# google/zopfli

Measured on AMD Instinct MI355X. Metric: input MB/s at numiterations=15 (gzip, bit-exact vs reference), higher is better.
Workload: dtype u8 (f32/f64 cost DP); 1 GPU; class-T synthetic (text-like, the enwik8 stand-in) 100000000 B per GPU, numiterations=15, blocksplitting=0, gzip, BASELINE configs[1]; total_bytes=100000000, master_blocks=100, gather=none (one rank)

## Files before the change

include/zopfli_amd.h:

```cpp
#ifndef ZOPFLI_AMD_H_
#define ZOPFLI_AMD_H_

#include <stddef.h>
#include <stdint.h>

#ifdef __cplusplus
extern "C" {
#endif

#if defined(__GNUC__)
#pragma GCC visibility push(default)
#endif



typedef struct ZopfliOptions {
  int verbose;
  int verbose_more;
  int numiterations;
  int blocksplitting;
  int blocksplittinglast;
  int blocksplittingmax;
} ZopfliOptions;

// ... 164 lines not shown
int zmx_master_block_costs(const unsigned char* in, size_t insize, double* cost, size_t ncost);
int zmx_deal_master_blocks(const double* cost, size_t nblocks, size_t shards, size_t* first);

int zmx_last_timing(double* out8);

int zmx_last_kernel_timing(double* out4);
void zmx_set_kernel_timing(int on);

int zmx_last_host_timing(double* out2);

int zmx_last_match_timing(double* out4);
int zmx_last_match_walk(double* out3);

typedef void (*zmx_oom_hook_t)(int device);
void zmx_set_oom_hook(zmx_oom_hook_t hook);
int zmx_ctx_set_share(zmx_ctx* ctx, unsigned contexts_on_device);
int zmx_ctx_trim_cache(zmx_ctx* ctx);
int zmx_ctx_set_priority(zmx_ctx* ctx, int level);

int zmx_set_match_kernel(int kernel);

int zmx_last_seg_stats(double* out8);

#if defined(__GNUC__)
#pragma GCC visibility pop
#endif

#ifdef __cplusplus
}
#endif

#endif
```

zopfli_amd/api.py:

```python
import ctypes
import os

from ._build import LIB

if os.environ.get("ZOPFLI_AMD_LIB"):
    LIB = os.environ["ZOPFLI_AMD_LIB"]

FORMAT_GZIP, FORMAT_ZLIB, FORMAT_DEFLATE = 0, 1, 2
CRC32, ADLER32 = 0, 1
ZMX_HIST = 320


class ZopfliOptions(ctypes.Structure):
    _fields_ = [("verbose", ctypes.c_int), ("verbose_more", ctypes.c_int), ("numiterations", ctypes.c_int),
                ("blocksplitting", ctypes.c_int), ("blocksplittinglast", ctypes.c_int),
                ("blocksplittingmax", ctypes.c_int)]

    def __init__(self, numiterations=15, blocksplitting=1, blocksplittingmax=15, verbose=0, verbose_more=0):
        super().__init__(verbose, verbose_more, numiterations, blocksplitting, 0, blocksplittingmax)


class ZmxBlock(ctypes.Structure):
    _fields_ = [("instart", ctypes.c_uint64), ("inend", ctypes.c_uint64)]

# ... 160 lines not shown
    k = (ctypes.c_double * 4)()
    lib.zmx_last_kernel_timing(k)
    d["wtab_kernel"], d["trace_kernel"] = k[0], k[2]
    h = (ctypes.c_double * 2)()
    lib.zmx_last_host_timing(h)
    d["download"], d["serialize"] = h[0], h[1]
    m = (ctypes.c_double * 4)()
    lib.zmx_last_match_timing(m)
    d["match_kernel"], d["hash_kernels"], d["table_builds"], d["positions_matched"] = m[0], m[1], m[2], m[3]
    w = (ctypes.c_double * 3)()
    lib.zmx_last_match_walk(w)
    d["skip_walk_lane_iterations"], d["skip_walk_wave_iterations"], d["skip_walk_positions"] = w[0], w[1], w[2]
    return d


def last_seg_stats(lib=None):
    lib = lib or library()
    t = (ctypes.c_double * 8)()
    lib.zmx_last_seg_stats(t)
    keys = ["tasks", "accepted", "rerun_state", "rerun_level", "rerun_tie", "positions_rerun", "rerun_values", "positions"]
    return dict(zip(keys, list(t)))


class Context:

    def __init__(self, device=0, lib=None):
        self.lib = lib or library()
        self.handle = ctypes.c_void_p()
        self._input = None
        self._segments = None
        if self.lib.zmx_ctx_create(device, ctypes.byref(self.handle)) != 0:
            raise RuntimeError("zmx_ctx_create: " + self.error())

    def error(self):
        return (self.lib.zmx_last_error() or b"").decode()

    def _check(self, rc, what):
        if rc != 0:
            raise RuntimeError(f"{what}: {self.error()}")

    def close(self):
        if self.handle:
            self.lib.zmx_ctx_destroy(self.handle)
            self.handle = ctypes.c_void_p()

    def set_input(self, data):
# ... 316 lines not shown
```

zopfli_amd/csrc/device/zmx_dp4.h:

```cpp
#pragma once

#define D3_RELAX_K(CS, LT, WV, K)                                            \
  {                                                                          \
    const double old_ = (double)(CS);                                        \
    const double nc_ = (WV) + cj;                                            \
    LT = nc_ < old_ ? (K) : LT;                                              \
    CS = (float)fmin(nc_, old_);                                             \
  }

#define D3_ROT32()                                                           \
  {                                                                          \
    if (reach < 64) {                    \
      c[0] = __uint_as_float(__builtin_amdgcn_permlane32_swap(__float_as_uint(c[0]), __float_as_uint(1e30f), false, false)[1]); \
      l[0] = __builtin_amdgcn_permlane32_swap(l[0], 0u, false, false)[1];    \
    } else {                                                                 \
      d3_rot32(c, l, lane);                                                  \
    }                                                                        \
    reach = reach >= 32 ? reach - 32 : 0;                                    \
  }

#define D4_TRACK_MAX() { vmax = fmaxf(vmax, c[0] < 1e29f ? c[0] : 0.0f); }

#define D3_RETIRE32(WB)                                                      \
  {                                                                          \
// ... 216 lines not shown
  u64* prof;
  const u32* badpos;
  const SegTask* tasks;
  const u32* task_off;
  float* lvl;
  const float* est_bits;
  SegSnap* entry;
  SegSnap* exit;
  SegSnap* mid;
  SegCheck* chk;
  const float* wmax;
  const u32* tiemask;
  u32* stats;
  float level_scale;
  const u32* wg_tasks;
  const u32* wmeta;
  const u32* winroff;
  const u32* winflag;
  const u32* win_off;
  int debug;
  u16* over;
  u32* redo_count;
  u32* redo_wg;
  int int_path;
  int fix_lean_min;
  int redo_pass;
  int chain_fast;
  int coop;
  const u32* kind;
  const u32* run_list;
  u32* flags;
};

struct D4Job {
  u32 cell = 0;
  u32 start;
  u32 noshort;
  u32 pout;
  u32 pend;
  u32 la_lo;
  u32 over_lo;
  bool spec;
  bool load;
  float level;
  double delta;
  const SegSnap* init;
// ... 486 lines not shown
            }
          }
        }
      }
      const u64 tk1 = D3_TICK();
      __syncthreads();
      if (PROF) { tq[2] += tk1 - tk0; tq[3] += D3_TICK() - tk1; }
      ++it;
      if (last) break;
    }
    __syncthreads();
    if (PROF && P.prof && wave == 2 && lane == 0) {
      u64* o = P.prof + (u64)b * ZMX_PROF_N + 24;
      for (int i = 0; i < 4; ++i) atomicAdd(&o[i], tq[i]);
    }
  }
#undef D3_TICK
  __builtin_amdgcn_fence(__ATOMIC_RELEASE, "agent");
  __syncthreads();
  __builtin_amdgcn_fence(__ATOMIC_ACQUIRE, "agent");
}

__global__ __launch_bounds__(64) void k_dpcheck(Dp4Params P) {
  if (blockIdx.x == 0 && threadIdx.x == 0) *P.redo_count = 0;
  const u32 t = P.task0 + blockIdx.x;
  if (P.tasks[t].pout == 0) return;
  const SegCheck r = d4_check(&P.exit[t - 1], &P.entry[t], threadIdx.x);
  if (threadIdx.x == 0) P.chk[t] = r;
}

__device__ __forceinline__ u32 d4_accept(float vmin, double vmax, double delta, double wmax, u32 tiemask) {
  if (delta == 0.0) return 0;
  const int e = (int)((__float_as_uint(vmin) >> 23) & 255u) - 127;
  const double lo = ldexp(1.0, e), hi = ldexp(1.0, e + 1);
  const bool pure = vmin >= 16.0f && vmax + wmax < hi && (double)vmin + delta >= lo && vmax + wmax + delta < hi;
  if (!pure) return 1;
  return ((tiemask >> (e & 31)) & 1u) != 0 ? 2u : 0u;
}

__global__ __launch_bounds__(64) void k_dpscan(Dp4Params P) {
  const u32 b = P.block0 + blockIdx.x;
  const u32 t0 = P.task_off[b], t1 = P.task_off[b + 1];
  const u32 lane = threadIdx.x;
  const double wmax = (double)P.wmax[b] + 1.0;
  const u32 tiemask = P.tiemask[b];
  double carry = 0.0;
  for (u32 c0 = t0 + 1; c0 < t1; c0 += 64) {
    const u32 t = c0 + lane;
    const bool act = t < t1;
    SegCheck ck;
    ck.d = 0.0; ck.vmin = 0.0f; ck.match = 0;
// ... 31 lines not shown
```

zopfli_amd/csrc/device/zmx_hip.hip:

```cpp
#include <hip/hip_runtime.h>

#include <algorithm>
#include <atomic>
#include <cmath>
#include <cstdio>
#include <cstdlib>
#include <cstring>
#include <mutex>
#include <string>
#include <unordered_map>
#include <vector>

#include "zmx_kernels.h"
#include "zmx_match2.h"
#ifdef ZMX_EXPERIMENTS
#include "zmx_match3.h"
#include "zmx_match4.h"
#else
#define BK_CH 32768u
#endif
#include "zmx_match5.h"
#include "zmx_dp4.h"
#include "zmx_dp5.h"
#include "zmx_encode.h"
#include "zmx_checksum.h"
#include "zmx_trace.h"
#include "zmx_greedy.h"
#include "zmx_png.h"
#include "zmx_png_brute.h"
#include "zmx_blockcost.h"
#include "zopfli_amd.h"
#include "../host/symbol_check.h"
#include "../host/thread_pool.h"

namespace {

thread_local std::string g_err;
struct ThreadStats {
  double kernel_seconds[3];
  double squeeze_launches;
  double match5[3];
  double match[4];
  double seg[8];
};
static_assert(sizeof(ThreadStats) == 19 * sizeof(double), "zmx_internal_stats_take / _add move 19 doubles");
thread_local ThreadStats g_ts = {};
#define g_kernel_seconds g_ts.kernel_seconds
#define g_squeeze_launches g_ts.squeeze_launches
#define g_match5_stats g_ts.match5
#define g_match_stats g_ts.match
#define g_seg_stats g_ts.seg

thread_local bool g_last_oom = false;
thread_local int g_err_class = ZMX_ERR_NONE;

int Fail(const char* what, hipError_t e, const char* file, int line) {
  char buf[512];
  std::snprintf(buf, sizeof(buf), "%s: %s (%s:%d)", what, hipGetErrorString(e), file, line);
  g_err = buf;
  g_last_oom = e == hipErrorOutOfMemory;
  g_err_class = g_last_oom ? ZMX_ERR_OUT_OF_MEMORY : ZMX_ERR_DEVICE;
  if (g_last_oom) (void)hipGetLastError();
  return -1;
}
int FailMsg(const std::string& m) {
  g_err = m;
  g_err_class = ZMX_ERR_REFUSED;
  return -1;
}
int FailFault(const std::string& m) {
  g_err = m;
  g_err_class = ZMX_ERR_DEVICE;
  return -1;
}
// ... 94 lines not shown
  bool buckets = false;
  u32* d_recs = nullptr;
  u32* d_pool = nullptr;
  u32 pool_cap = 0;
  u16* d_la = nullptr;
  u32* d_store[2] = {nullptr, nullptr};
  u32* d_hist = nullptr;
  u32* d_nsym = nullptr;
  double* d_cost = nullptr;
  double* d_mincost = nullptr;
  int* d_slot = nullptr;
  uint2* d_dph = nullptr;
  u64* d_block_edges = nullptr;
  u32* d_badpos = nullptr;
  size_t badpos_words = 0;
  bool badpos_clean = false;
  u64* d_code_base = nullptr;
  u16* d_codes = nullptr;
  double* d_wtab = nullptr;
  u32* d_badcodes = nullptr;
  u32* d_seg_off = nullptr;
  u32* d_extab = nullptr;
  uint2* d_seginfo = nullptr;
  std::vector<u32> seg_off;
  std::vector<u64> block_edges;
  std::vector<u32> tile_off;
  u32* d_counters = nullptr;
  u32* d_flags = nullptr;
  unsigned char* d_runin = nullptr;
  unsigned char* d_runout = nullptr;
  unsigned char* h_runin = nullptr;
  unsigned char* h_runout = nullptr;
  size_t h_runin_cap = 0, h_runout_cap = 0;
  size_t runin_bytes = 0, runout_bytes = 0;
  u64* d_prof = nullptr;
  std::vector<SegTask> tasks;
  std::vector<u32> task_off;
  SegTask* d_tasks = nullptr;
  u32* d_task_off = nullptr;
  u32* d_wg_tasks = nullptr;
  u32 n_wg = 0;
  u32 n_wg_runs = 0;
  u32* d_task_kind = nullptr;
  u32* d_run_list = nullptr;
  u32 n_run_list = 0;
  u32* d_wmeta = nullptr;
// ... 251 lines not shown
  c->pool_free_bytes = 0;
  return 0;
}

int zmx_set_match_kernel(int kernel) {
#ifdef ZMX_EXPERIMENTS
  if (kernel != 0 && kernel != 2 && kernel != 3 && kernel != 4 && kernel != 5) return FailMsg("zmx_set_match_kernel: 0, 2, 3, 4 or 5");
#else
  if (kernel == 3 || kernel == 4) return FailMsg("zmx_set_match_kernel: kernels 3 and 4 are in -DZMX_EXPERIMENTS builds only");
  if (kernel != 0 && kernel != 2 && kernel != 5) return FailMsg("zmx_set_match_kernel: 0, 2 or 5");
#endif
  g_match_kernel.store(kernel, std::memory_order_relaxed);
  return 0;
}

size_t zmx_internal_input_size(zmx_ctx* ctx) { return ctx->insize; }
int zmx_internal_device(zmx_ctx* ctx) { return ctx->device; }
void zmx_internal_set_error(const char* msg) { g_err = msg; g_err_class = ZMX_ERR_DEVICE; }
void zmx_internal_set_error_class(const char* msg, int cls) { g_err = msg; g_err_class = cls; }
const unsigned char* zmx_internal_input_host(zmx_ctx* ctx) { return ctx->h_in; }

void zmx_internal_seg_stats(double* out8, int reset) {
  for (int i = 0; i < 8; ++i) out8[i] = g_seg_stats[i];
  if (reset) for (int i = 0; i < 8; ++i) g_seg_stats[i] = 0;
}

void zmx_internal_match5_stats(double* out3, int reset) {
  for (int i = 0; i < 3; ++i) out3[i] = g_match5_stats[i];
  if (reset) for (int i = 0; i < 3; ++i) g_match5_stats[i] = 0;
}

void zmx_internal_match_stats(double* out4, int reset) {
  for (int i = 0; i < 4; ++i) out4[i] = g_match_stats[i];
  if (reset) for (int i = 0; i < 4; ++i) g_match_stats[i] = 0;
}

void zmx_internal_kernel_stats(double* seconds3, double* squeeze_launches, int reset) {
  for (int i = 0; i < 3; ++i) seconds3[i] = g_kernel_seconds[i];
  *squeeze_launches = g_squeeze_launches;
  if (reset) {
    g_kernel_seconds[0] = g_kernel_seconds[1] = g_kernel_seconds[2] = 0;
    g_squeeze_launches = 0;
  }
}

void zmx_internal_stats_take(double* out19) {
  std::memcpy(out19, &g_ts, sizeof(g_ts));
  g_ts = ThreadStats{};
}
void zmx_internal_stats_add(const double* in19) {
  double* d = reinterpret_cast<double*>(&g_ts);
  for (int i = 0; i < 19; ++i) d[i] += in19[i];
}

static hipError_t PinnedTake(zmx_ctx* c, unsigned char** p, size_t bytes, size_t* cap) {
  size_t best = c->pinned_free.size();
  for (size_t i = 0; i < c->pinned_free.size(); ++i) {
    const size_t k = c->pinned_free[i].second;
    if (k >= bytes && k <= 4 * bytes + 4096 && (best == c->pinned_free.size() || k < c->pinned_free[best].second)) best = i;
  }
  if (best != c->pinned_free.size()) {
    *p = c->pinned_free[best].first;
    *cap = c->pinned_free[best].second;
    c->pinned_free.erase(c->pinned_free.begin() + static_cast<long>(best));
    return hipSuccess;
  }
  *cap = bytes < 4096 ? 4096 : bytes;
  return hipHostMalloc(reinterpret_cast<void**>(p), *cap, hipHostMallocDefault);
}
static void PinnedGive(zmx_ctx* c, unsigned char** p, size_t cap) {
  if (!*p) return;
  if (c && c->pinned_free.size() < 8 && cap <= (64u << 20)) c->pinned_free.emplace_back(*p, cap);
  else (void)hipHostFree(*p);
  *p = nullptr;
}
// ... 105 lines not shown

static void ReleaseTableArrays(zmx_ctx* c, zmx_tables* t, bool keep_stores) {
  auto rel = [&](auto*& p) { PoolFree(c, p); p = nullptr; };
  rel(t->d_blocks);
  rel(t->d_tile_off);
  rel(t->d_same16);
  rel(t->d_links);
  rel(t->d_sorted_alloc);
  rel(t->d_ssame);
  rel(t->d_chunk_base);
  rel(t->d_recs);
  rel(t->d_pool);
  rel(t->d_la);
  rel(t->d_dph);
  rel(t->d_block_edges);
  rel(t->d_badpos);
  rel(t->d_code_base);
  rel(t->d_codes);
  rel(t->d_wtab);
  rel(t->d_badcodes);
  rel(t->d_seg_off);
  rel(t->d_extab);
  rel(t->d_seginfo);
  rel(t->d_counters);
  rel(t->d_prof);
  rel(t->d_tasks);
  rel(t->d_task_off);
  rel(t->d_wg_tasks);
  rel(t->d_task_kind);
  rel(t->d_run_list);
  rel(t->d_wmeta);
  rel(t->d_runin);
  rel(t->d_runout);
  rel(t->d_winroff);
  rel(t->d_winflag);
  rel(t->d_win_off);
  rel(t->d_lvl);
  rel(t->d_entry);
  rel(t->d_exit);
  rel(t->d_mid);
  rel(t->d_chk);
  rel(t->d_over);
  rel(t->d_redo);
  for (int h = 0; h < 2; ++h) { rel(t->d_rank[h]); rel(t->d_bucket[h]); }
  t->d_sorted[0] = t->d_sorted[1] = nullptr;
  PinnedGive(c, &t->h_runin, t->h_runin_cap);
// ... 16 lines not shown
  HIPCHK(hipStreamSynchronize(c->stream));
  HIPCHK(hipStreamSynchronize(c->stream2));
  ReleaseTableArrays(c, t, true);
  t->trimmed = true;
  return 0;
}

static unsigned EnvU32(const char* name, unsigned dflt, unsigned lo, unsigned hi) {
  const char* e = std::getenv(name);
  if (!e) return dflt;
  const long v = std::atol(e);
  return v < static_cast<long>(lo) ? lo : v > static_cast<long>(hi) ? hi : static_cast<unsigned>(v);
}
static unsigned SegL(u64 total_positions) {
  static const bool set = std::getenv("ZOPFLI_AMD_SEG_L") != nullptr;
  static const unsigned v = EnvU32("ZOPFLI_AMD_SEG_L", 4096, 0, 1u << 24) & ~63u;
  if (set) return v;
  return total_positions <= (128u << 10) ? 256u : total_positions <= (16u << 20) ? 512u : total_positions <= (48u << 20) ? 1024u : 2048u;
}
static unsigned SegHead(size_t nb) {
  static const unsigned v = EnvU32("ZOPFLI_AMD_SEG_HEAD", 0, 0, 1u << 24) & ~63u;
  return v ? v : (nb >= 48 ? 8192u : 0u);
}
static unsigned SegWarm() { static const unsigned v = (EnvU32("ZOPFLI_AMD_SEG_WARM", 512, 64, 1u << 20) + 63u) & ~63u; return v; }

static int BuildTables(zmx_ctx* c, const zmx_block* blocks, size_t nb, zmx_tables* t, zmx_tables* parent = nullptr, bool with_dp = true) {
  const int mk = MatchKernel();
  t->matches_only = !with_dp;
  t->nb = nb;
  t->blocks.resize(nb);
  t->bsize.resize(nb);
  t->store_begin[0].assign(nb, 0);
  t->store_begin[1].assign(nb, 0);
  std::vector<u32> tile_off(nb + 1, 0);
  u64 pos_off = 0, reg_off = 0, la_off = 0, max_l = 0;
  for (size_t b = 0; b < nb; ++b) {
    if (blocks[b].inend < blocks[b].instart || blocks[b].inend > c->insize) {
      return FailMsg("zmx_tables_build: block outside the resident input");
    }
    BlockDesc& d = t->blocks[b];
    d.instart = blocks[b].instart;
    d.inend = blocks[b].inend;
    d.ws = d.instart > ZMX_WINDOW ? d.instart - ZMX_WINDOW : 0;
    if (!c->seg_starts.empty()) {
      const size_t k = static_cast<size_t>(std::upper_bound(c->seg_starts.begin(), c->seg_starts.end(), d.instart) -
                                           c->seg_starts.begin()) - 1;
// ... 649 lines not shown
        const u32 Bk = t->bsize[T.block];
        return (T.pend < Bk ? T.pend : Bk) - T.q;
      };
      std::stable_sort(runs.begin(), runs.end(), [&](u32 a, u32 b2) { return walked(a) > walked(b2); });
      t->n_run_list = static_cast<u32>(runs.size());
      HIPCHK(PoolAlloc(c, &t->d_task_kind, ntk + 4));
      HIPCHK(PoolAlloc(c, &t->d_run_list, runs.size() + 4));
      if (ntk) HIPCHK(hipMemcpyAsync(t->d_task_kind, kind.data(), ntk * sizeof(u32), hipMemcpyHostToDevice, c->stream));
      if (!runs.empty()) HIPCHK(hipMemcpyAsync(t->d_run_list, runs.data(), runs.size() * sizeof(u32), hipMemcpyHostToDevice, c->stream));
      HIPCHK(hipStreamSynchronize(c->stream));
    }
    wg.insert(wg.end(), wg_runs.begin(), wg_runs.end());
    HIPCHK(PoolAlloc(c, &t->d_wg_tasks, wg.size() + 4));
    if (!wg.empty()) HIPCHK(hipMemcpyAsync(t->d_wg_tasks, wg.data(), wg.size() * sizeof(u32), hipMemcpyHostToDevice, c->stream));
    HIPCHK(hipStreamSynchronize(c->stream));
  }
  }
  t->seg_off.assign(nb + 1, 0);
  for (size_t b = 0; b < nb; ++b) t->seg_off[b + 1] = t->seg_off[b] + (t->bsize[b] + TS_SEG - 1) / TS_SEG;
  HIPCHK(PoolAlloc(c, &t->d_seg_off, nb + 1));
  HIPCHK(PoolAlloc(c, &t->d_extab, static_cast<size_t>(t->seg_off[nb]) * GS_STATES));
  HIPCHK(PoolAlloc(c, &t->d_seginfo, t->seg_off[nb]));
  HIPCHK(hipMemcpyAsync(t->d_seg_off, t->seg_off.data(), (nb + 1) * sizeof(u32), hipMemcpyHostToDevice, c->stream));
  HIPCHK(hipStreamSynchronize(c->stream));
  return 0;
}

int zmx_tables_build(zmx_ctx* c, const zmx_block* blocks, size_t nblocks, zmx_tables** out) {
  return zmx_tables_build_from(c, nullptr, blocks, nblocks, out);
}

int zmx_tables_build_matches(zmx_ctx* c, const zmx_block* blocks, size_t nblocks, zmx_tables** out) {
  DeviceGuard dev_guard(c->device);
  HIPCHK(dev_guard.err);
  zmx_tables* t = new zmx_tables();
  g_last_oom = false;
  const int rc = BuildTables(c, blocks, nblocks, t, nullptr, false);
  if (rc) {
    zmx_tables_free(c, t);
    return rc == -1 && g_last_oom && nblocks > 1 ? kTooLarge : rc;
  }
  *out = t;
  return 0;
}

int zmx_tables_build_from(zmx_ctx* c, zmx_tables* parent, const zmx_block* blocks, size_t nblocks, zmx_tables** out) {
  if (parent && parent->trimmed) return FailMsg("zmx_tables_build_from: these tables were trimmed to their stores (zmx_tables_trim)");
// ... 178 lines not shown
  cp.est_bits = t->squeeze_runs == 0 ? t->d_runinfo + 2 * nb : nullptr;
  cp.entry = t->d_entry;
  cp.exit = t->d_exit;
  static const bool mid_on = EnvU32("ZOPFLI_AMD_SEG_MID", 1, 0, 1) != 0;
  cp.mid = mid_on ? t->d_mid : nullptr;
  cp.chk = t->d_chk;
  cp.over = t->d_over;
  cp.wmax = t->d_runinfo;
  cp.tiemask = reinterpret_cast<const u32*>(t->d_runinfo + nb);
  cp.stats = t->d_segstats;
  static const float level_scale = [] { const char* e = std::getenv("ZOPFLI_AMD_SEG_SCALE"); return e ? static_cast<float>(std::atof(e)) : 1.0f; }();
  cp.level_scale = level_scale;
  cp.wg_tasks = t->d_wg_tasks;
  static const int seg_debug = [] { const char* e = std::getenv("ZOPFLI_AMD_SEG_DEBUG"); return e ? std::atoi(e) : 0; }();
  cp.debug = seg_debug;
  static const int fix_lean = [] { const char* e = std::getenv("ZOPFLI_AMD_FIX_LEAN"); return e ? std::atoi(e) : -1; }();
  cp.fix_lean_min = fix_lean;
  static const int int_path = [] { const char* e = std::getenv("ZOPFLI_AMD_INT_PATH"); return e ? std::atoi(e) : 1; }();
  cp.int_path = int_path;
  static const int chain_fast = [] { const char* e = std::getenv("ZOPFLI_AMD_SHORTCUT_CHAIN"); return e ? std::atoi(e) : 1; }();
  cp.chain_fast = chain_fast;
  cp.redo_count = t->d_redo;
  cp.redo_wg = t->d_redo + 4;
  cp.redo_pass = 0;
#ifdef ZMX_EXPERIMENTS
  static const int coop = [] { const char* e = std::getenv("ZOPFLI_AMD_COOP"); return e ? std::atoi(e) : 0; }();
#else
  constexpr int coop = 0;
#endif
  cp.coop = coop != 0 ? 1 : 0;
  cp.kind = t->d_task_kind;
  cp.run_list = t->d_run_list;
  cp.flags = t->d_flags;
  cp.wmeta = t->d_wmeta;
  cp.winroff = t->d_winroff;
  cp.winflag = t->d_winflag;
  cp.win_off = t->d_win_off;
  const bool scan_bad = any_below_mincost;
  if (scan_bad || !t->badpos_clean) HIPCHK(hipMemsetAsync(t->d_badpos, 0, t->badpos_words * sizeof(u32), c->stream));
  t->badpos_clean = !scan_bad;
  TraceSegParams tp;
  tp.blocks = t->d_blocks;
  tp.seg_off = t->d_seg_off;
  tp.nb_total = static_cast<u32>(nb);
  tp.recs = t->d_recs;
  tp.pool = t->d_pool;
  tp.la = t->d_la;
  tp.slot = t->d_slot;
  tp.store0 = t->d_store[0];
  tp.store1 = t->d_store[1];
  tp.hist_out = t->d_hist;
  tp.nsym_out = t->d_nsym;
  tp.flags = t->d_flags;
  tp.extab = t->d_extab;
  tp.seginfo = t->d_seginfo;
  tp.block0 = 0;
  tp.seg0 = 0;
  double ksec[3] = {0, 0, 0};
  const bool timing = KernelTiming();
  const dim3 dpdim(64 * (D3_NB + 2));
  {
    const unsigned nblk = static_cast<unsigned>(nb);
    const unsigned tiles = t->tile_off[nb];
    const unsigned ntask = t->task_off[nb];
    if (timing) HIPCHK(hipEventRecord(c->ev[0], c->stream));
    hipLaunchKernelGGL(k_wtab, dim3(nblk), dim3(256), 0, c->stream, wp);
    KCHK(c, "k_wtab");
    if (tiles && scan_bad) hipLaunchKernelGGL(k_badscan, dim3(tiles), dim3(256), 0, c->stream, bp);
    KCHK(c, "k_badscan");
    HIPCHK(hipGetLastError());
    if (timing) HIPCHK(hipEventRecord(c->ev[1], c->stream));
    {
      const dim3 bdim(64 * D5_WG);
      if (t->n_wg_runs) {
        HIPCHK(hipEventRecord(c->ev2[0], c->stream));
        HIPCHK(hipStreamWaitEvent(c->stream2, c->ev2[0], 0));
        Dp4Params cr = cp;
        cr.task0 = t->n_wg;
// ... 1 lines not shown
        if (cp.coop && cp.prof) hipLaunchKernelGGL((k_dp6_spec<2, true>), dim3(t->n_run_list), dim3(64 * D6_NW), 0, c->stream2, cr);
        else if (cp.coop) hipLaunchKernelGGL((k_dp6_spec<2, false>), dim3(t->n_run_list), dim3(64 * D6_NW), 0, c->stream2, cr);
        else
#endif
        if (cp.prof) hipLaunchKernelGGL((k_dp5_spec<true, 2, true>), dim3(t->n_wg_runs), bdim, 0, c->stream2, cr);
        else hipLaunchKernelGGL((k_dp5_spec<false, 2, true>), dim3(t->n_wg_runs), bdim, 0, c->stream2, cr);
        HIPCHK(hipGetLastError());
        HIPCHK(hipEventRecord(c->ev2[1], c->stream2));
      }
      if (t->n_wg) {
        if (cp.prof) hipLaunchKernelGGL((k_dp5_spec<true, 4, false>), dim3(t->n_wg), bdim, 0, c->stream, cp);
        else hipLaunchKernelGGL((k_dp5_spec<false, 4, false>), dim3(t->n_wg), bdim, 0, c->stream, cp);
        HIPCHK(hipGetLastError());
      }
      if (t->n_wg_runs) HIPCHK(hipStreamWaitEvent(c->stream, c->ev2[1], 0));
      if (GuardOn()) HIPCHK(hipStreamSynchronize(c->stream2));
      KCHK(c, "k_dp5_spec");
    }
    if (ntask > nblk) {
      hipLaunchKernelGGL(k_dpcheck, dim3(ntask), dim3(64), 0, c->stream, cp);
      KCHK(c, "k_dpcheck");
      static const int redo = [] { const char* e = std::getenv("ZOPFLI_AMD_SEG_REDO"); return e ? std::atoi(e) : 1; }();
      for (int pass = 0; pass < redo; ++pass) {
        hipLaunchKernelGGL(k_dpscan, dim3(nblk), dim3(64), 0, c->stream, cp);
        KCHK(c, "k_dpscan");
        Dp4Params c2 = cp;
        c2.redo_pass = 1;
        c2.est_bits = nullptr;
        const unsigned cap = ntask;
#ifdef ZMX_EXPERIMENTS
        if (t->n_wg_runs && cp.coop) {
          hipLaunchKernelGGL((k_dp6_spec<2, false>), dim3(cap), dim3(64 * D6_NW), 0, c->stream, c2);
          if (cp.prof) hipLaunchKernelGGL((k_dp5_spec<true, 4, false>), dim3(cap), dim3(64 * D5_WG), 0, c->stream, c2);
          else hipLaunchKernelGGL((k_dp5_spec<false, 4, false>), dim3(cap), dim3(64 * D5_WG), 0, c->stream, c2);
        } else
#endif
        if (t->n_wg_runs) {
          if (cp.prof) hipLaunchKernelGGL((k_dp5_spec<true, 2, true>), dim3(cap), dim3(64 * D5_WG), 0, c->stream, c2);
          else hipLaunchKernelGGL((k_dp5_spec<false, 2, true>), dim3(cap), dim3(64 * D5_WG), 0, c->stream, c2);
        } else {
          if (cp.prof) hipLaunchKernelGGL((k_dp5_spec<true, 4, false>), dim3(cap), dim3(64 * D5_WG), 0, c->stream, c2);
          else hipLaunchKernelGGL((k_dp5_spec<false, 4, false>), dim3(cap), dim3(64 * D5_WG), 0, c->stream, c2);
        }
        KCHK(c, "k_dp5_spec");
        hipLaunchKernelGGL(k_dpcheck, dim3(ntask), dim3(64), 0, c->stream, cp);
        KCHK(c, "k_dpcheck");
      }
      if (cp.prof) hipLaunchKernelGGL(k_dp4_fix<true>, dim3(nblk), dpdim, 0, c->stream, cp);
      else hipLaunchKernelGGL(k_dp4_fix<false>, dim3(nblk), dpdim, 0, c->stream, cp);
      KCHK(c, "k_dp4_fix");
    }
    HIPCHK(hipGetLastError());
    if (timing) HIPCHK(hipEventRecord(c->ev[2], c->stream));
    const unsigned nseg = t->seg_off[nb];
    if (nseg) hipLaunchKernelGGL(k_trace_exits, dim3(nseg), dim3(TS_THREADS), 0, c->stream, tp);
    KCHK(c, "k_trace_exits");
    hipLaunchKernelGGL(k_trace_link, dim3(nblk), dim3(64), 0, c->stream, tp);
    KCHK(c, "k_trace_link");
    if (nseg) hipLaunchKernelGGL(k_trace_emit, dim3(nseg), dim3(64), 0, c->stream, tp);
    KCHK(c, "k_trace_emit");
    HIPCHK(hipGetLastError());
    if (timing) HIPCHK(hipEventRecord(c->ev[3], c->stream));
  }
  u32 segstats[8];
  HIPCHK(hipMemcpyAsync(t->h_runout, t->d_runout, t->runout_bytes, hipMemcpyDeviceToHost, c->stream));
  HIPCHK(hipStreamSynchronize(c->stream));
  for (int i = 0; i < 3 && timing; ++i) {
    float ms = 0;
    HIPCHK(hipEventElapsedTime(&ms, c->ev[i], c->ev[i + 1]));
    ksec[i] += ms * 1e-3;
  }
  {
    const u32* o_hist = reinterpret_cast<const u32*>(t->h_runout);
    const u32* o_nsym = o_hist + nb * ZMX_HIST;
    const u32* o_stats = o_nsym + nb;
    const u32* o_flags = o_stats + 8;
    std::memcpy(hist, o_hist, nb * ZMX_HIST * sizeof(u32));
    std::memcpy(nsym, o_nsym, nb * sizeof(u32));
    std::memcpy(segstats, o_stats, sizeof(segstats));
    if (o_flags[1]) {
      char buf[128];
      std::snprintf(buf, sizeof(buf), "zmx_squeeze_run: device consistency flags 0x%x", o_flags[1]);
      return FailFault(buf);
    }
  }
  t->h_hist.assign(hist, hist + nb * ZMX_HIST);
  t->have_hist = true;
  ++t->squeeze_runs;
  {
    for (int i = 0; i < 3; ++i) g_kernel_seconds[i] += ksec[i];
    g_squeeze_launches += 1;
    for (int i = 0; i < 7; ++i) g_seg_stats[i] += segstats[i];
    g_seg_stats[7] += static_cast<double>(t->total_b);
  }
  for (size_t b = 0; b < nb; ++b) t->store_begin[slot[b]][b] = t->bsize[b] - nsym[b];
  if (t->d_prof) {
    std::vector<u64> pr(nb * ZMX_PROF_N);
    HIPCHK(hipMemcpy(pr.data(), t->d_prof, pr.size() * sizeof(u64), hipMemcpyDeviceToHost));
    double a[ZMX_PROF_N] = {};
    for (size_t b = 0; b < nb; ++b)
      for (unsigned k = 0; k < ZMX_PROF_N; ++k) a[k] += static_cast<double>(pr[b * ZMX_PROF_N + k]);
    if (cp.coop && t->n_run_list) {
      double mxj = 0;
      for (size_t b = 0; b < nb; ++b) mxj = std::max(mxj, static_cast<double>(pr[b * ZMX_PROF_N + 16]));
      std::fprintf(stderr, "coop prof (k_dp6_spec, first pass, wave 0): job cycles %.3g (longest job %.3g): token+flow %.3g, class 1 %.3g, class 2 %.3g, "
                   "headers %.3g, other stretches %.3g (%.0f positions, %.0f each), run stretches %.3g (%.0f positions, %.0f each), general step %.3g (%.0f, %.0f each), "
                   "shortcuts %.3g (%.0f, %.0f each), waiting for wave 1 at the rotation %.3g (%.0f windows, %.0f each); wave 1: %.3g of %.3g cycles inside get()\n",
                   a[9], mxj, a[0], a[1], a[2], a[3], a[4], a[10], a[4] / (a[10] + 1e-9), a[5], a[11], a[5] / (a[11] + 1e-9), a[6], a[12], a[6] / (a[12] + 1e-9),
                   a[7], a[13], a[7] / (a[13] + 1e-9), a[8], a[14], a[8] / (a[14] + 1e-9), a[15], a[17]);
    }
    std::fprintf(stderr, "squeeze prof: edges %.2f ms chain %.2f ms trace %.2f ms; chain wave busy %.1f cycles/position, "
                 "%.0f steps, fast %.1f%% of %.0f positions walked (%zu in the blocks); tasks %u accepted %u re-run "
                 "state %u values %u level %u tie %u (%u positions, %u by the lean job)\n",
                 ksec[0] * 1e3, ksec[1] * 1e3, ksec[2] * 1e3, a[1] / a[4], a[0],
                 100.0 * a[2] / (a[2] + a[3] + 1e-9), a[4], t->total_b, segstats[0], segstats[1], segstats[2],
                 segstats[6], segstats[3], segstats[4], segstats[5], segstats[7]);
// ... 792 lines not shown
```

zopfli_amd/csrc/device/zmx_trace.h:

```cpp
#pragma once

#define TS_SEG 4096u
#define TS_ENT 258u

struct TraceSegParams {
  const BlockDesc* blocks;
  const u32* seg_off;
  u32 nb_total;
  u32 block0;
  u32 seg0;
  const u32* recs;
  const u32* pool;
  const u16* la;
  const int* slot;
  u32* store0;
  u32* store1;
  u32* hist_out;
  u32* nsym_out;
  u32* flags;
  u32* extab;
  uint2* seginfo;
};

__device__ __forceinline__ void ts_bounds(u32 B, u32 s, u32& lo, u32& hi) {
  hi = B - s * TS_SEG;
  lo = hi > TS_SEG ? hi - TS_SEG : 0u;
}

__device__ __forceinline__ u32 ts_find_block(const u32* seg_off, u32 nb, u32 seg) {
  u32 lo = 0, hi = nb;
  while (hi - lo > 1) {
    const u32 mid = (lo + hi) >> 1;
    if (seg_off[mid] <= seg) lo = mid; else hi = mid;
  }
  return lo;
}

#define TS_ROUNDS 6
#define TS_THREADS 512u

__global__ __launch_bounds__(TS_THREADS) void k_trace_exits(TraceSegParams P) {
  __shared__ u32 s_j[TS_SEG + 1];
  const u32 seg = P.seg0 + blockIdx.x;
  const u32 b = ts_find_block(P.seg_off, P.nb_total, seg);
  const BlockDesc bd = P.blocks[b];
  const u32 B = (u32)(bd.inend - bd.instart);
  u32 lo, hi;
  ts_bounds(B, seg - P.seg_off[b], lo, hi);
  const u16* la = P.la + bd.la_off;
  const u32 n = hi - lo;
  for (u32 x = threadIdx.x + 1; x <= n; x += TS_THREADS) {
    const u32 h = lo + x;
    u32 len = la[h];
    if (len == 0) len = 1;
    if (len > h) len = h;
    const u32 t = h - len;
    s_j[x] = (t > lo ? t - lo : 0x8000u | (lo - t)) | (1u << 16);
  }
  __syncthreads();
  for (int r = 0; r < TS_ROUNDS; ++r) {
    for (u32 x = threadIdx.x + 1; x <= n; x += TS_THREADS) {
      const u32 v = s_j[x];
      if (!(v & 0x8000u)) {
        const u32 w = s_j[v & 0xffffu];
        s_j[x] = (w & 0xffffu) | ((v & 0xffff0000u) + (w & 0xffff0000u));
      }
    }
    __syncthreads();
  }
  const u32 j = threadIdx.x;
  if (j < TS_ENT && n > j) {
    u32 v = s_j[n - j];
    while (!(v & 0x8000u)) {
      const u32 w = s_j[v & 0xffffu];
      v = (w & 0xffffu) | ((v & 0xffff0000u) + (w & 0xffff0000u));
    }
    P.extab[(u64)seg * TS_ENT + j] = (v & 0x7fffu) | (v & 0xffff0000u);
  }
}

__global__ __launch_bounds__(64) void k_trace_link(TraceSegParams P) {
  const u32 b = P.block0 + blockIdx.x;
  const BlockDesc bd = P.blocks[b];
  const u32 B = (u32)(bd.inend - bd.instart);
  const u32 lane = threadIdx.x;
  for (u32 i = lane; i < 320; i += 64) P.hist_out[(u64)b * 320 + i] = 0;
  if (lane != 0) return;
  const u32 s0 = P.seg_off[b], ns = P.seg_off[b + 1] - s0;
  u32 j = 0, off = 0;
  for (u32 s = 0; s < ns; ++s) {
    P.seginfo[s0 + s] = make_uint2(j, off);
    u32 lo, hi;
    ts_bounds(B, s, lo, hi);
    if (hi - lo <= j) {
      P.seginfo[s0 + s] = make_uint2(0xffffffffu, off);
      continue;
    }
    const u32 v = P.extab[(u64)(s0 + s) * TS_ENT + j];
    off += v >> 16;
    j = v & 0xffffu;
  }
  P.nsym_out[b] = off;
}

__global__ __launch_bounds__(64) void k_trace_emit(TraceSegParams P) {
  __shared__ __align__(16) u16 s_la[TR_CHUNK];
  __shared__ u32 s_sym[128];
  __shared__ u32 s_len[128];
  __shared__ u32 s_hist[320];

  const u32 seg = P.seg0 + blockIdx.x;
  const u32 b = ts_find_block(P.seg_off, P.nb_total, seg);
  const BlockDesc bd = P.blocks[b];
  const u32 B = (u32)(bd.inend - bd.instart);
  const u32 lane = threadIdx.x;
  u32 seg_lo, seg_hi;
  ts_bounds(B, seg - P.seg_off[b], seg_lo, seg_hi);
  const uint2 info = P.seginfo[seg];
  const u32* rbase = P.recs + bd.pos_off * 8;
  const u16* la = P.la + bd.la_off;
  u32* sbase = (P.slot[b] ? P.store1 : P.store0) + bd.pos_off;

  for (u32 i = lane; i < 320; i += 64) s_hist[i] = 0;
  __syncthreads();

  u32 head = seg_hi - info.x;
  if (seg_hi - seg_lo <= info.x) head = seg_lo;
  u32 total = info.y;
  u32 queued = 0;
  u32 lo = 0, hi = 0;
  bool bad = false;
  u32 pend_n = 0, pend_total = 0, pend_len = 0;
  uint4 pend_ra = make_uint4(0, 0, 0, 0), pend_rb = make_uint4(0, 0, 0, 0);

  for (;;) {
    while (queued < 64 && head > seg_lo && !bad) {
      const u32 wb = head > 63 ? head - 63 : 0;
      if (hi == 0 || wb < lo) {
        lo = head > TR_CHUNK - 8 ? (head - (TR_CHUNK - 8)) & ~7u : 0;
        hi = head;
        __syncthreads();
        uint4 v[4];
#pragma unroll
        for (int r = 0; r < 4; ++r) {
          const u32 i8 = (lane + 64u * r) * 8;
          v[r] = make_uint4(0, 0, 0, 0);
          if (lo + i8 <= hi) v[r] = *reinterpret_cast<const uint4*>(la + lo + i8);
        }
#pragma unroll
        for (int r = 0; r < 4; ++r) reinterpret_cast<uint4*>(s_la)[lane + 64 * r] = v[r];
// ... 44 lines not shown
              const u32 mid = (plo + phi) >> 1;
              if ((P.pool[off + mid] & 0xffffu) < pend_len) plo = mid + 1; else phi = mid;
            }
            if (plo < cnt) dist = P.pool[off + plo] >> 16;
          }
          e = pend_len | (dist << 16);
          if (dist == 0) atomicOr(&P.flags[1], 4u);
        } else {
          e = (d1 >> 16) & 255u;
        }
        sbase[B - 1 - (pend_total + lane)] = e;
        hist_add_symbol(s_hist, e & 0xffffu, e >> 16);
      }
      pend_n = 0;
    }
    if (queued == 0) break;
    {
      const u32 n = queued < 64 ? queued : 64;
      pend_n = n;
      pend_total = total;
      if (lane < n) {
        const u32 pos = s_sym[lane];
        pend_len = s_len[lane];
        const u32* rec = rbase + (u64)pos * 8;
        pend_ra = *reinterpret_cast<const uint4*>(rec);
        pend_rb = *reinterpret_cast<const uint4*>(rec + 4);
      }
      total += n;
      const u32 rest = queued - n;
      __syncthreads();
      u32 mv_s = 0, mv_l = 0;
      if (lane < rest) { mv_s = s_sym[n + lane]; mv_l = s_len[n + lane]; }
      __syncthreads();
      if (lane < rest) { s_sym[lane] = mv_s; s_len[lane] = mv_l; }
      queued = rest;
      __syncthreads();
    }
  }
  if (bad && lane == 0) atomicOr(&P.flags[1], 2u);
  __syncthreads();
  for (u32 i = lane; i < 320; i += 64) {
    const u32 v = s_hist[i];
    if (v) atomicAdd(&P.hist_out[(u64)b * 320 + i], v);
  }
}
```

zopfli_amd/csrc/host/api.cc:

```cpp
#include <chrono>
#include <malloc.h>
#include <cstdio>
#include <cstdlib>
#include <cstring>
#include <algorithm>
#include <condition_variable>
#include <memory>
#include <mutex>
#include <string>
#include <thread>
#include <unordered_map>
#include <vector>

#include "block_cache.h"
#include "block_cost.h"
#include "deflate.h"
#include "lz77_optimal.h"
#include "symbols.h"
#include "deal.h"
#include "dealing.h"
#include "thread_pool.h"
#include "zopfli_amd.h"

extern "C" void zmx_internal_kernel_stats(double* seconds3, double* squeeze_launches, int reset);
extern "C" void zmx_internal_seg_stats(double* out8, int reset);
extern "C" void zmx_internal_match_stats(double* out4, int reset);
extern "C" void zmx_internal_match5_stats(double* out3, int reset);
extern "C" void zmx_internal_stats_take(double* out19);
extern "C" void zmx_internal_stats_add(const double* in19);
extern "C" size_t zmx_internal_input_size(zmx_ctx* ctx);
extern "C" const unsigned char* zmx_internal_input_host(zmx_ctx* ctx);
extern "C" void zmx_internal_set_error(const char* msg);

namespace {

using zamd::kMasterBlock;

[[noreturn]] void Die(const char* what) {
  std::fprintf(stderr, "zopfli_amd: %s: %s\n", what, zmx_last_error());
  std::exit(EXIT_FAILURE);
}

void MaybeKeepHeap() {
  static const bool once = [] {
    const char* e = std::getenv("ZOPFLI_AMD_KEEP_HEAP");
    if (!e || std::atoi(e) == 0) return true;
    if (std::atoi(e) == 2) {
      mallopt(M_MMAP_THRESHOLD, 32 << 20);
      mallopt(M_TRIM_THRESHOLD, 1 << 30);
      mallopt(M_TOP_PAD, 64 << 20);
    } else {
      mallopt(M_TRIM_THRESHOLD, 1 << 30);
// ... 293 lines not shown
  }
  const double tr_begin = WallMs();
  const Lease lease(parts.size(), split_from && parts.size() >= split_from && !one_context ? split_ways : 1,
                    parts.size() < 32, parts.size() < 32);
  const double tr_lease = WallMs();
  struct InlineHostWork {
    bool on, was;
    explicit InlineHostWork(bool o) : on(o), was(zamd::g_host_inline) { if (on) zamd::g_host_inline = true; }
    ~InlineHostWork() { if (on) zamd::g_host_inline = was; }
  } inline_host(parts.size() <= 2 && Pool().InFlight() > 1);
  const std::vector<zmx_ctx*>& ctxs = lease.ctxs;
  const size_t ndev = std::min(ctxs.size(), parts.size());
  struct Shard {
    size_t first = 0, last = 0, base = 0;
    std::vector<zamd::Chunk> chunks;
    std::vector<size_t> part_chunks;
    int rc = 0;
    std::string err;
    int err_class = ZMX_ERR_NONE;
    zamd::Timing timing;
    uint32_t sum = 0;
    size_t sum_bytes = 0;
    bool redone = false;
    double stats[19] = {0};
  };
  std::vector<Shard> shards(ndev);
  for (size_t d = 0; d < ndev; ++d) {
    shards[d].first = parts.size() * d / ndev;
    shards[d].last = parts.size() * (d + 1) / ndev;
  }
  static const bool deal_by_cost = [] { const char* e = std::getenv("ZOPFLI_AMD_DEAL"); return !e || std::strcmp(e, "count") != 0; }();
  if (deal_by_cost && ndev > 1 && in != nullptr && parts.size() > ndev) {
    std::vector<double> cost(parts.size());
    zamd::ParallelFor(parts.size(), [&](size_t i) { cost[i] = zamd::MasterBlockCost(in, parts[i].instart, parts[i].inend); });
    std::vector<size_t> first;
    zamd::DealByCost(cost, ndev, &first);
    for (size_t d = 0; d < ndev; ++d) { shards[d].first = first[d]; shards[d].last = first[d + 1]; }
  }
  if (const char* e = std::getenv("ZOPFLI_AMD_SHARD_WEIGHTS")) {
    std::vector<double> w;
    for (const char* q = e; *q;) {
      char* end = nullptr;
      const double v = std::strtod(q, &end);
      if (end == q) break;
      w.push_back(v > 0 ? v : 0);
      q = *end == ',' ? end + 1 : end;
    }
// ... 471 lines not shown
```

Before: 806.0 MB/s.

## Precompute trace cut points so blocks trace segments independently, and compact redo checks

Adds a table-build kernel that finds, for each trace segment, a position no match can straddle, so the backward trace of the squeeze path can start at known cut points instead of running the per-segment exit tables. Blocks where every segment has a cut use a new count kernel plus a prefix-sum link, while other blocks keep the old exit-table trace over a compacted segment list. It also replaces the full-grid redo check with a kernel that visits only the redone tasks, using double-buffered redo counters, and skips the match record load for literal symbols. The cost is extra table-build work, a host sync and download per table build, and more code paths that must stay bit-exact.

```diff
diff --git a/include/zopfli_amd.h b/include/zopfli_amd.h
--- a/include/zopfli_amd.h
+++ b/include/zopfli_amd.h
@@ -210,6 +210,8 @@
 
 int zmx_last_seg_stats(double* out8);
 
+int zmx_last_trace_stats(double* out4, int reset);
+
 #if defined(__GNUC__)
 #pragma GCC visibility pop
 #endif
diff --git a/zopfli_amd/api.py b/zopfli_amd/api.py
--- a/zopfli_amd/api.py
+++ b/zopfli_amd/api.py
@@ -206,6 +206,16 @@
     return dict(zip(keys, list(t)))
 
 
+def last_trace_stats(lib=None, reset=False):
+    lib = lib or library()
+    fn = lib.zmx_last_trace_stats
+    fn.argtypes = [ctypes.POINTER(ctypes.c_double), ctypes.c_int]
+    t = (ctypes.c_double * 4)()
+    fn(t, 1 if reset else 0)
+    keys = ["cut_blocks", "cut_segments", "table_blocks", "table_segments"]
+    return dict(zip(keys, list(t)))
+
+
 class Context:
 
     def __init__(self, device=0, lib=None):
diff --git a/zopfli_amd/csrc/device/zmx_dp4.h b/zopfli_amd/csrc/device/zmx_dp4.h
--- a/zopfli_amd/csrc/device/zmx_dp4.h
+++ b/zopfli_amd/csrc/device/zmx_dp4.h
@@ -262,6 +262,7 @@
   u16* over;
   u32* redo_count;
   u32* redo_wg;
+  u32* redo_next;
   int int_path;
   int fix_lean_min;
   int redo_pass;
@@ -794,11 +795,25 @@
 }
 
 __global__ __launch_bounds__(64) void k_dpcheck(Dp4Params P) {
-  if (blockIdx.x == 0 && threadIdx.x == 0) *P.redo_count = 0;
+  if (blockIdx.x == 0 && threadIdx.x == 0) { P.redo_count[0] = 0; P.redo_count[1] = 0; }
   const u32 t = P.task0 + blockIdx.x;
   if (P.tasks[t].pout == 0) return;
   const SegCheck r = d4_check(&P.exit[t - 1], &P.entry[t], threadIdx.x);
   if (threadIdx.x == 0) P.chk[t] = r;
+}
+
+__global__ __launch_bounds__(128) void k_dpcheck_redo(Dp4Params P) {
+  if (blockIdx.x == 0 && threadIdx.x == 0) *P.redo_next = 0;
+  const u32 n = *P.redo_count;
+  const u32 wave = threadIdx.x >> 6, lane = threadIdx.x & 63;
+  for (u32 i = blockIdx.x; i < n; i += gridDim.x) {
+    const u32 t0 = P.redo_wg[(u64)i * 4];
+    const u32 t = t0 + wave;
+    if (wave != 0 && t >= P.task_off[P.tasks[t0].block + 1]) continue;
+    if (P.tasks[t].pout == 0) continue;
+    const SegCheck r = d4_check(&P.exit[t - 1], &P.entry[t], lane);
+    if (lane == 0) P.chk[t] = r;
+  }
 }
 
 __device__ __forceinline__ u32 d4_accept(float vmin, double vmax, double delta, double wmax, u32 tiemask) {
diff --git a/zopfli_amd/csrc/device/zmx_hip.hip b/zopfli_amd/csrc/device/zmx_hip.hip
--- a/zopfli_amd/csrc/device/zmx_hip.hip
+++ b/zopfli_amd/csrc/device/zmx_hip.hip
@@ -42,14 +42,16 @@
   double match5[3];
   double match[4];
   double seg[8];
+  double trace[4];
 };
-static_assert(sizeof(ThreadStats) == 19 * sizeof(double), "zmx_internal_stats_take / _add move 19 doubles");
+static_assert(sizeof(ThreadStats) == 23 * sizeof(double), "zmx_internal_stats_take / _add move 23 doubles");
 thread_local ThreadStats g_ts = {};
 #define g_kernel_seconds g_ts.kernel_seconds
 #define g_squeeze_launches g_ts.squeeze_launches
 #define g_match5_stats g_ts.match5
 #define g_match_stats g_ts.match
 #define g_seg_stats g_ts.seg
+#define g_trace_stats g_ts.trace
 
 thread_local bool g_last_oom = false;
 thread_local int g_err_class = ZMX_ERR_NONE;
@@ -190,6 +192,11 @@
   u32* d_seg_off = nullptr;
   u32* d_extab = nullptr;
   uint2* d_seginfo = nullptr;
+  u32* d_seg_entry = nullptr;
+  u32* d_blk_cut = nullptr;
+  u32* d_seg_cnt = nullptr;
+  u32* d_tab_segs = nullptr;
+  u32 n_tab_segs = 0, n_cut_blocks = 0;
   std::vector<u32> seg_off;
   std::vector<u64> block_edges;
   std::vector<u32> tile_off;
@@ -487,7 +494,16 @@
 
 void zmx_internal_seg_stats(double* out8, int reset) {
   for (int i = 0; i < 8; ++i) out8[i] = g_seg_stats[i];
-  if (reset) for (int i = 0; i < 8; ++i) g_seg_stats[i] = 0;
+  if (reset) {
+    for (int i = 0; i < 8; ++i) g_seg_stats[i] = 0;
+    for (int i = 0; i < 4; ++i) g_trace_stats[i] = 0;
+  }
+}
+
+int zmx_last_trace_stats(double* out4, int reset) {
+  for (int i = 0; i < 4; ++i) out4[i] = g_trace_stats[i];
+  if (reset) for (int i = 0; i < 4; ++i) g_trace_stats[i] = 0;
+  return 0;
 }
 
 void zmx_internal_match5_stats(double* out3, int reset) {
@@ -509,13 +525,13 @@
   }
 }
 
-void zmx_internal_stats_take(double* out19) {
-  std::memcpy(out19, &g_ts, sizeof(g_ts));
+void zmx_internal_stats_take(double* out23) {
+  std::memcpy(out23, &g_ts, sizeof(g_ts));
   g_ts = ThreadStats{};
 }
-void zmx_internal_stats_add(const double* in19) {
+void zmx_internal_stats_add(const double* in23) {
   double* d = reinterpret_cast<double*>(&g_ts);
-  for (int i = 0; i < 19; ++i) d[i] += in19[i];
+  for (int i = 0; i < 23; ++i) d[i] += in23[i];
 }
 
 static hipError_t PinnedTake(zmx_ctx* c, unsigned char** p, size_t bytes, size_t* cap) {
@@ -667,6 +683,10 @@
   rel(t->d_seg_off);
   rel(t->d_extab);
   rel(t->d_seginfo);
+  rel(t->d_seg_entry);
+  rel(t->d_blk_cut);
+  rel(t->d_seg_cnt);
+  rel(t->d_tab_segs);
   rel(t->d_counters);
   rel(t->d_prof);
   rel(t->d_tasks);
@@ -729,6 +749,7 @@
   static const unsigned v = EnvU32("ZOPFLI_AMD_SEG_HEAD", 0, 0, 1u << 24) & ~63u;
   return v ? v : (nb >= 48 ? 8192u : 0u);
 }
+static bool TraceCuts() { static const bool v = EnvU32("ZOPFLI_AMD_TRACE_CUTS", 1, 0, 1) != 0; return v; }
 static unsigned SegWarm() { static const unsigned v = (EnvU32("ZOPFLI_AMD_SEG_WARM", 512, 64, 1u << 20) + 63u) & ~63u; return v; }
 
 static int BuildTables(zmx_ctx* c, const zmx_block* blocks, size_t nb, zmx_tables* t, zmx_tables* parent = nullptr, bool with_dp = true) {
@@ -1424,7 +1445,41 @@
   HIPCHK(PoolAlloc(c, &t->d_extab, static_cast<size_t>(t->seg_off[nb]) * GS_STATES));
   HIPCHK(PoolAlloc(c, &t->d_seginfo, t->seg_off[nb]));
   HIPCHK(hipMemcpyAsync(t->d_seg_off, t->seg_off.data(), (nb + 1) * sizeof(u32), hipMemcpyHostToDevice, c->stream));
-  HIPCHK(hipStreamSynchronize(c->stream));
+  {
+    const u32 nseg = t->seg_off[nb];
+    HIPCHK(PoolAlloc(c, &t->d_seg_entry, nseg + 1));
+    HIPCHK(PoolAlloc(c, &t->d_seg_cnt, nseg + 1));
+    HIPCHK(PoolAlloc(c, &t->d_blk_cut, nb));
+    std::vector<u32> blk_cut(nb, 0);
+    if (TraceCuts() && with_dp && nseg) {
+      HIPCHK(hipMemsetD32Async(reinterpret_cast<hipDeviceptr_t>(t->d_blk_cut), 1, nb, c->stream));
+      TraceCutParams xp;
+      xp.blocks = t->d_blocks;
+      xp.dph = t->d_dph;
+      xp.seg_off = t->d_seg_off;
+      xp.nb = static_cast<u32>(nb);
+      xp.seg_entry = t->d_seg_entry;
+      xp.blk_cut = t->d_blk_cut;
+      hipLaunchKernelGGL(k_trace_cuts, dim3(nseg), dim3(64), 0, c->stream, xp);
+      KCHK(c, "k_trace_cuts");
+      HIPCHK(hipMemcpyAsync(blk_cut.data(), t->d_blk_cut, nb * sizeof(u32), hipMemcpyDeviceToHost, c->stream));
+    } else {
+      HIPCHK(hipMemsetAsync(t->d_blk_cut, 0, nb * sizeof(u32), c->stream));
+    }
+    HIPCHK(hipStreamSynchronize(c->stream));
+    std::vector<u32> tab_segs;
+    t->n_cut_blocks = 0;
+    for (size_t b = 0; b < nb; ++b) {
+      if (blk_cut[b]) { ++t->n_cut_blocks; continue; }
+      for (u32 s = t->seg_off[b]; s < t->seg_off[b + 1]; ++s) tab_segs.push_back(s);
+    }
+    t->n_tab_segs = static_cast<u32>(tab_segs.size());
+    HIPCHK(PoolAlloc(c, &t->d_tab_segs, tab_segs.size() + 1));
+    if (!tab_segs.empty()) {
+      HIPCHK(hipMemcpyAsync(t->d_tab_segs, tab_segs.data(), tab_segs.size() * sizeof(u32), hipMemcpyHostToDevice, c->stream));
+      HIPCHK(hipStreamSynchronize(c->stream));
+    }
+  }
   return 0;
 }
 
@@ -1649,6 +1704,7 @@
   cp.chain_fast = chain_fast;
   cp.redo_count = t->d_redo;
   cp.redo_wg = t->d_redo + 4;
+  cp.redo_next = t->d_redo + 1;
   cp.redo_pass = 0;
 #ifdef ZMX_EXPERIMENTS
   static const int coop = [] { const char* e = std::getenv("ZOPFLI_AMD_COOP"); return e ? std::atoi(e) : 0; }();
@@ -1681,6 +1737,11 @@
   tp.flags = t->d_flags;
   tp.extab = t->d_extab;
   tp.seginfo = t->d_seginfo;
+  tp.in = c->d_in;
+  tp.blk_cut = t->d_blk_cut;
+  tp.seg_entry = t->d_seg_entry;
+  tp.seg_cnt = t->d_seg_cnt;
+  tp.tab_segs = t->d_tab_segs;
   tp.block0 = 0;
   tp.seg0 = 0;
   double ksec[3] = {0, 0, 0};
@@ -1728,9 +1789,12 @@
       KCHK(c, "k_dpcheck");
       static const int redo = [] { const char* e = std::getenv("ZOPFLI_AMD_SEG_REDO"); return e ? std::atoi(e) : 1; }();
       for (int pass = 0; pass < redo; ++pass) {
-        hipLaunchKernelGGL(k_dpscan, dim3(nblk), dim3(64), 0, c->stream, cp);
+        Dp4Params cl = cp;
+        cl.redo_count = t->d_redo + (pass & 1);
+        cl.redo_next = t->d_redo + ((pass + 1) & 1);
+        hipLaunchKernelGGL(k_dpscan, dim3(nblk), dim3(64), 0, c->stream, cl);
         KCHK(c, "k_dpscan");
-        Dp4Params c2 = cp;
+        Dp4Params c2 = cl;
         c2.redo_pass = 1;
         c2.est_bits = nullptr;
         const unsigned cap = ntask;
@@ -1749,8 +1813,8 @@
           else hipLaunchKernelGGL((k_dp5_spec<false, 4, false>), dim3(cap), dim3(64 * D5_WG), 0, c->stream, c2);
         }
         KCHK(c, "k_dp5_spec");
-        hipLaunchKernelGGL(k_dpcheck, dim3(ntask), dim3(64), 0, c->stream, cp);
-        KCHK(c, "k_dpcheck");
+        hipLaunchKernelGGL(k_dpcheck_redo, dim3(std::min(ntask, 256u)), dim3(128), 0, c->stream, cl);
+        KCHK(c, "k_dpcheck_redo");
       }
       if (cp.prof) hipLaunchKernelGGL(k_dp4_fix<true>, dim3(nblk), dpdim, 0, c->stream, cp);
       else hipLaunchKernelGGL(k_dp4_fix<false>, dim3(nblk), dpdim, 0, c->stream, cp);
@@ -1759,7 +1823,9 @@
     HIPCHK(hipGetLastError());
     if (timing) HIPCHK(hipEventRecord(c->ev[2], c->stream));
     const unsigned nseg = t->seg_off[nb];
-    if (nseg) hipLaunchKernelGGL(k_trace_exits, dim3(nseg), dim3(TS_THREADS), 0, c->stream, tp);
+    if (t->n_cut_blocks && nseg) hipLaunchKernelGGL(k_trace_count, dim3(nseg), dim3(64), 0, c->stream, tp);
+    KCHK(c, "k_trace_count");
+    if (t->n_tab_segs) hipLaunchKernelGGL(k_trace_exits, dim3(t->n_tab_segs), dim3(TS_THREADS), 0, c->stream, tp);
     KCHK(c, "k_trace_exits");
     hipLaunchKernelGGL(k_trace_link, dim3(nblk), dim3(64), 0, c->stream, tp);
     KCHK(c, "k_trace_link");
@@ -1798,6 +1864,10 @@
     g_squeeze_launches += 1;
     for (int i = 0; i < 7; ++i) g_seg_stats[i] += segstats[i];
     g_seg_stats[7] += static_cast<double>(t->total_b);
+    g_trace_stats[0] += t->n_cut_blocks;
+    g_trace_stats[1] += t->seg_off[nb] - t->n_tab_segs;
+    g_trace_stats[2] += static_cast<double>(nb - t->n_cut_blocks);
+    g_trace_stats[3] += t->n_tab_segs;
   }
   for (size_t b = 0; b < nb; ++b) t->store_begin[slot[b]][b] = t->bsize[b] - nsym[b];
   if (t->d_prof) {
diff --git a/zopfli_amd/csrc/device/zmx_trace.h b/zopfli_amd/csrc/device/zmx_trace.h
--- a/zopfli_amd/csrc/device/zmx_trace.h
+++ b/zopfli_amd/csrc/device/zmx_trace.h
@@ -20,6 +20,11 @@
   u32* flags;
   u32* extab;
   uint2* seginfo;
+  const u8* in;
+  const u32* blk_cut;
+  const u32* seg_entry;
+  u32* seg_cnt;
+  const u32* tab_segs;
 };
 
 __device__ __forceinline__ void ts_bounds(u32 B, u32 s, u32& lo, u32& hi) {
@@ -41,7 +46,7 @@
 
 __global__ __launch_bounds__(TS_THREADS) void k_trace_exits(TraceSegParams P) {
   __shared__ u32 s_j[TS_SEG + 1];
-  const u32 seg = P.seg0 + blockIdx.x;
+  const u32 seg = P.tab_segs[blockIdx.x];
   const u32 b = ts_find_block(P.seg_off, P.nb_total, seg);
   const BlockDesc bd = P.blocks[b];
   const u32 B = (u32)(bd.inend - bd.instart);
@@ -79,14 +84,131 @@
   }
 }
 
+struct TraceCutParams {
+  const BlockDesc* blocks;
+  const uint2* dph;
+  const u32* seg_off;
+  u32 nb;
+  u32* seg_entry;
+  u32* blk_cut;
+};
+
+#define TC_STRETCH 512u
+#define TC_LOADS ((TC_STRETCH + ZMX_MAX_MATCH + 63u) / 64u)
+
+__global__ __launch_bounds__(64) void k_trace_cuts(TraceCutParams P) {
+  const u32 seg = blockIdx.x;
+  const u32 b = ts_find_block(P.seg_off, P.nb, seg);
+  const BlockDesc bd = P.blocks[b];
+  const u32 B = (u32)(bd.inend - bd.instart);
+  const u32 s = seg - P.seg_off[b];
+  const u32 lane = threadIdx.x;
+  if (s == 0) {
+    if (lane == 0) P.seg_entry[seg] = B;
+    return;
+  }
+  const uint2* dph = P.dph + bd.pos_off;
+  const u32 x = B - s * TS_SEG;
+  const u32 xn = x > TS_SEG ? x - TS_SEG : 0u;
+  u32 best = 0;
+  for (u32 top = x; top > xn && best == 0;) {
+    const u32 bot = top - xn > TC_STRETCH ? top - TC_STRETCH : xn;
+    const u32 lo = bot + 1 > ZMX_MAX_MATCH ? bot + 1 - ZMX_MAX_MATCH : 0u;
+    u32 r[TC_LOADS];
+#pragma unroll
+    for (u32 i = 0; i < TC_LOADS; ++i) {
+      const u32 p = lo + 64u * i + lane;
+      r[i] = p < top ? p + (dph[p].y & 0xffffu) : 0u;
+    }
+    u32 carry = 0;
+#pragma unroll
+    for (u32 i = 0; i < TC_LOADS; ++i) {
+      const u32 p = lo + 64u * i + lane;
+      u32 incl = wave_scan_max(r[i]);
+      incl = incl > carry ? incl : carry;
+      const u64 ok = __ballot(p < top && p + 1 > bot && incl <= p + 1);
+      if (ok) best = lo + 64u * i + (63u - (u32)__builtin_clzll(ok)) + 1u;
+      carry = rdlane_u32(incl, 63);
+    }
+    top = bot;
+  }
+  if (lane == 0) {
+    P.seg_entry[seg] = best;
+    if (best == 0 && xn != 0) P.blk_cut[b] = 0;
+  }
+}
+
+__global__ __launch_bounds__(64) void k_trace_count(TraceSegParams P) {
+  __shared__ __align__(16) u16 s_la[TR_CHUNK];
+  const u32 seg = P.seg0 + blockIdx.x;
+  const u32 b = ts_find_block(P.seg_off, P.nb_total, seg);
+  if (!P.blk_cut[b]) return;
+  const BlockDesc bd = P.blocks[b];
+  const u32 lane = threadIdx.x;
+  const u16* la = P.la + bd.la_off;
+  u32 head = P.seg_entry[seg];
+  const u32 seg_lo = seg + 1 < P.seg_off[b + 1] ? P.seg_entry[seg + 1] : 0u;
+  u32 count = 0;
+  u32 lo = 0, hi = 0;
+  bool bad = false;
+  while (head > seg_lo) {
+    const u32 wb = head > 63 ? head - 63 : 0;
+    if (hi == 0 || wb < lo) {
+      lo = head > TR_CHUNK - 8 ? (head - (TR_CHUNK - 8)) & ~7u : 0;
+      hi = head;
+      __syncthreads();
+      uint4 v[4];
+#pragma unroll
+      for (int r = 0; r < 4; ++r) {
+        const u32 i8 = (lane + 64u * r) * 8;
+        v[r] = make_uint4(0, 0, 0, 0);
+        if (lo + i8 <= hi) v[r] = *reinterpret_cast<const uint4*>(la + lo + i8);
+      }
+#pragma unroll
+      for (int r = 0; r < 4; ++r) reinterpret_cast<uint4*>(s_la)[lane + 64 * r] = v[r];
+      __syncthreads();
+    }
+    const u32 cell = wb + lane;
+    const u32 la_raw = cell <= head ? (u32)s_la[cell - lo] : 0u;
+    const u32 la_v = la_raw ? la_raw : 1u;
+    u64 mask = 0;
+    int idx = (int)(head - wb);
+    const int lim = __builtin_amdgcn_readfirstlane((int)(seg_lo + 1 > wb ? seg_lo + 1 - wb : 0u));
+    do {
+      const u32 len = rdlane_u32(la_v, (u32)idx);
+      mask |= 1ull << idx;
+      idx -= (int)len;
+    } while (idx >= lim);
+    if (__ballot(((mask >> lane) & 1) && (la_raw == 0 || la_raw > cell))) { bad = true; break; }
+    head = (u32)((int)wb + idx);
+    count += (u32)__popcll(mask);
+  }
+  if (lane == 0) {
+    P.seg_cnt[seg] = count;
+    if (bad || head != seg_lo) atomicOr(&P.flags[1], 8u);
+  }
+}
+
 __global__ __launch_bounds__(64) void k_trace_link(TraceSegParams P) {
   const u32 b = P.block0 + blockIdx.x;
   const BlockDesc bd = P.blocks[b];
   const u32 B = (u32)(bd.inend - bd.instart);
   const u32 lane = threadIdx.x;
   for (u32 i = lane; i < 320; i += 64) P.hist_out[(u64)b * 320 + i] = 0;
+  const u32 s0 = P.seg_off[b], ns = P.seg_off[b + 1] - s0;
+  if (P.blk_cut[b]) {
+    u32 carry = 0;
+    for (u32 c0 = 0; c0 < ns; c0 += 64) {
+      const u32 s = c0 + lane;
+      const u32 v = s < ns ? P.seg_cnt[s0 + s] : 0u;
+      const u32 incl = wave_scan_add(v);
+      if (s < ns) P.seginfo[s0 + s] = make_uint2(0u, carry + incl - v);
+      carry += rdlane_u32(incl, 63);
+    }
+    if (lane == 0) P.nsym_out[b] = carry;
+    return;
+  }
   if (lane != 0) return;
-  const u32 s0 = P.seg_off[b], ns = P.seg_off[b + 1] - s0;
   u32 j = 0, off = 0;
   for (u32 s = 0; s < ns; ++s) {
     P.seginfo[s0 + s] = make_uint2(j, off);
@@ -126,6 +248,10 @@
 
   u32 head = seg_hi - info.x;
   if (seg_hi - seg_lo <= info.x) head = seg_lo;
+  if (P.blk_cut[b]) {
+    head = P.seg_entry[seg];
+    seg_lo = seg + 1 < P.seg_off[b + 1] ? P.seg_entry[seg + 1] : 0u;
+  }
   u32 total = info.y;
   u32 queued = 0;
   u32 lo = 0, hi = 0;
@@ -216,9 +342,13 @@
       if (lane < n) {
         const u32 pos = s_sym[lane];
         pend_len = s_len[lane];
-        const u32* rec = rbase + (u64)pos * 8;
-        pend_ra = *reinterpret_cast<const uint4*>(rec);
-        pend_rb = *reinterpret_cast<const uint4*>(rec + 4);
+        if (pend_len >= 3) {
+          const u32* rec = rbase + (u64)pos * 8;
+          pend_ra = *reinterpret_cast<const uint4*>(rec);
+          pend_rb = *reinterpret_cast<const uint4*>(rec + 4);
+        } else {
+          pend_ra.y = (u32)P.in[bd.instart + pos] << 16;
+        }
       }
       total += n;
       const u32 rest = queued - n;
diff --git a/zopfli_amd/csrc/host/api.cc b/zopfli_amd/csrc/host/api.cc
--- a/zopfli_amd/csrc/host/api.cc
+++ b/zopfli_amd/csrc/host/api.cc
@@ -26,8 +26,8 @@
 extern "C" void zmx_internal_seg_stats(double* out8, int reset);
 extern "C" void zmx_internal_match_stats(double* out4, int reset);
 extern "C" void zmx_internal_match5_stats(double* out3, int reset);
-extern "C" void zmx_internal_stats_take(double* out19);
-extern "C" void zmx_internal_stats_add(const double* in19);
+extern "C" void zmx_internal_stats_take(double* out23);
+extern "C" void zmx_internal_stats_add(const double* in23);
 extern "C" size_t zmx_internal_input_size(zmx_ctx* ctx);
 extern "C" const unsigned char* zmx_internal_input_host(zmx_ctx* ctx);
 extern "C" void zmx_internal_set_error(const char* msg);
@@ -367,7 +367,7 @@
     uint32_t sum = 0;
     size_t sum_bytes = 0;
     bool redone = false;
-    double stats[19] = {0};
+    double stats[23] = {0};
   };
   std::vector<Shard> shards(ndev);
   for (size_t d = 0; d < ndev; ++d) {
```

Measured after the change: 819.5 MB/s (median of 6 runs). No clear change (+1.7%).
